# mojing1999/jmcodec

Hardware: AMD Instinct MI355X
Metric: decoded frames/sec @1080p H.264 + bit-exact YUV (higher is better)
Workload: dtype u8

## Files before the change

### jmcodec_amd/csrc/intra_lds.hip

```cpp
#include <hip/hip_runtime.h>
#include "jobs.h"
#include "kernels.h"
#include "kernel_common.h"
#include "chain_common.h"
#include "intra_device.h"

namespace jmamd {

__global__ __launch_bounds__(kIBandRows * 16) __attribute__((amdgpu_waves_per_eu(1, 2))) void k_intra_band(const PicParams *pics, int *ctl, int *err) {
    __shared__ __align__(16) uint8_t smem[kIntraSmemBytes];
    const PicParams &pp = pics[blockIdx.y];
    if (!(pp.stages & PS_INTRA_LDS)) return;
    intra_band_body<false>(pp, blockIdx.x >> 1, blockIdx.x & 1, ctl + (size_t)blockIdx.y * kChainStride + kChainIntraRing, smem, nullptr, err + blockIdx.y);
}

bool intra_lds_supported(int mb_w, int mb_h) { return mb_w > 0 && mb_h <= kIBandRows * kDeblockMaxBands; }

void launch_intra_lds(const PicParams *d_pics, int n, int max_mb_h, int *ctl, int *err, hipStream_t st) {
    const int bands = (max_mb_h + kIBandRows - 1) / kIBandRows;
    hipLaunchKernelGGL(k_intra_band, dim3(2 * bands, n), dim3(kIBandRows * 16), 0, st, d_pics, ctl, err);
}

}
```

Before: 15180.

## Prefetch intra macroblock inputs through a register ring and batch band progress publishing

Replaces the generic intra band body with a stage-pipelined version. Per-macroblock records, residuals and neighbour pixels are requested DEPTH wavefront steps ahead into a register ring, hiding global load latency behind reconstruction. Inter-band progress is now published only every PUB steps, which cuts atomic store and wait traffic but makes the band below wait a little longer. It adds register pressure and a more complex synchronisation protocol that has to stay bit-exact.

```diff
diff --git a/jmcodec_amd/csrc/intra_band_sched.h b/jmcodec_amd/csrc/intra_band_sched.h
--- /dev/null
+++ b/jmcodec_amd/csrc/intra_band_sched.h
@@ -0,0 +1,42 @@
+#pragma once
+#include <stdint.h>
+#ifndef JM_HD
+#if defined(__HIPCC__)
+#include <hip/hip_runtime.h>
+#define JM_HD __host__ __device__ __forceinline__
+#else
+#define JM_HD static inline
+#endif
+#endif
+
+namespace jmamd {
+namespace ibs {
+
+constexpr int kRows = 16;
+constexpr int kAllDone = 0x7fffffff;
+
+JM_HD int band_row0(int band) { return band * kRows; }
+JM_HD int band_rows(int mb_h, int band) { const int left = mb_h - band * kRows; return left < 0 ? 0 : (left < kRows ? left : kRows); }
+JM_HD int first_step(int band) { return 2 * band_row0(band); }
+JM_HD int last_step(int mb_w, int mb_h, int band) { return mb_w - 1 + 2 * (band_row0(band) + band_rows(mb_h, band) - 1); }
+
+JM_HD int mb_x(int s, int row) { return s - 2 * row; }
+JM_HD bool has_mb(int s, int row, int mb_w) { const int x = mb_x(s, row); return x >= 0 && x < mb_w; }
+
+JM_HD constexpr int ring_slots(int D) { return D + 1; }
+JM_HD constexpr int slot_of(int s, int first, int D) { return (s - first) % ring_slots(D); }
+JM_HD constexpr int requested_in(int s, int D) { return s + D; }
+constexpr int kMinDepth = 2, kMaxDepth = 3;
+JM_HD int request_x(int s, int row, int mb_w) { const int x = mb_x(s, row); return x < 0 ? 0 : (x < mb_w ? x : mb_w - 1); }
+JM_HD int group_row(int row0, int rows, int g) { return row0 + (g < rows ? g : 0); }
+
+JM_HD int store_step(int xm, int row0) { return xm + 2 * (row0 - 1); }
+JM_HD int need_above(int xm, int row0) { return store_step(xm, row0) + 1; }
+JM_HD bool covers(int v, int t) { return v > t; }
+JM_HD bool publishes(int s, int first, int P) { return (s - first) % P == 0; }
+JM_HD int published_in(int s) { return s; }
+JM_HD int published_after(int s, int first, int P) { return s - (s - first) % P; }
+JM_HD int publish_lag(int t, int first, int P) { return P - (t - first) % P; }
+
+}
+}
diff --git a/jmcodec_amd/csrc/intra_lds.hip b/jmcodec_amd/csrc/intra_lds.hip
--- a/jmcodec_amd/csrc/intra_lds.hip
+++ b/jmcodec_amd/csrc/intra_lds.hip
@@ -4,21 +4,142 @@
 #include "kernel_common.h"
 #include "chain_common.h"
 #include "intra_device.h"
+#include "intra_band_sched.h"
 
 namespace jmamd {
 
-__global__ __launch_bounds__(kIBandRows * 16) __attribute__((amdgpu_waves_per_eu(1, 2))) void k_intra_band(const PicParams *pics, int *ctl, int *err) {
+static_assert(ibs::kRows == kIBandRows, "intra_band_sched.h describes bands of kIBandRows rows");
+
+struct IStage { uint32_t rec, right; uint4 res0, res1, bot; };
+
+template <bool CHROMA>
+__device__ __forceinline__ IStage istage_request(const gbyte *mbs, const gbyte *resid, const gbyte *plane, int pitch, int mb_w, int row, int s, int l) {
+    constexpr int rows_per_mb = CHROMA ? 8 : 16;
+    const int x = ibs::request_x(s, row, mb_w);
+    const int mb = row * mb_w + x, my_row = CHROMA ? (l & 7) : l;
+    IStage st;
+    st.rec = gload1(mbs + (size_t)mb * sizeof(MbRec) + (l & 7) * 4);
+    const gbyte *px = plane + (size_t)(row * rows_per_mb) * pitch + x * 16;
+    const gbyte *rs = resid + (size_t)mb * 768;
+    st.right = gload1(px + (size_t)my_row * pitch + 12);
+    st.bot = gload4(px + (size_t)(rows_per_mb - 1) * pitch);
+    if (CHROMA) { st.res0 = gload4(rs + 512 + l * 16); st.res1 = make_uint4(0, 0, 0, 0); }
+    else { st.res0 = gload4(rs + l * 32); st.res1 = gload4(rs + l * 32 + 16); }
+    return st;
+}
+
+template <int DEPTH, bool CHROMA>
+__device__ __forceinline__ void intra_stage_body(const PicParams &pp, int band, int *prog_pic, int pub, uint8_t *smem, int *err_word) {
+    const int mb_w = pp.mb_w, mb_h = pp.mb_h, pitch = pp.pitch;
+    const int rows = ibs::band_rows(mb_h, band);
+    if (rows <= 0) return;
+    const int row0 = ibs::band_row0(band);
+    int *prog = prog_pic + (CHROMA ? kDeblockMaxBands : 0);
+    const gbyte *resid = (const gbyte *)pp.resid;
+    const gbyte *mbs = (const gbyte *)pp.mbs;
+    ILds lds{smem, kIBandRows + 1};
+    const int g = threadIdx.x >> 4, l = threadIdx.x & 15;
+    const bool active = g < rows;
+    const int row = ibs::group_row(row0, rows, g), lrow = g + 1;
+    if (threadIdx.x < 144) { lds.i4tab()[threadIdx.x] = (uint8_t)i4_table_entry(threadIdx.x >> 4, threadIdx.x & 3, (threadIdx.x >> 2) & 3);
+        ((uint2 *)lds.i4sel())[threadIdx.x] = i4_sel_entry(threadIdx.x >> 4, threadIdx.x & 3, (threadIdx.x >> 2) & 3); }
+    if (!CHROMA && threadIdx.x < 144) ((pk::I8Sel *)lds.i8sel())[threadIdx.x] = pk::i8_sel_entry(threadIdx.x >> 4, threadIdx.x & 15);
+    gbyte *plane = (gbyte *)(cur_plane(pp) + (CHROMA ? pp.chroma_offset : 0));
+    const ICtx cx{plane, pitch};
+    constexpr int rows_per_mb = CHROMA ? 8 : 16;
+    const bool takes_ring = band > 0 && g == 0;
+    const bool gives_ring = active && g == rows - 1 && row < mb_h - 1;
+    const bool pub_wave = __builtin_amdgcn_readfirstlane((int)(threadIdx.x >> 6)) == ((rows - 1) >> 2) && row0 + rows < mb_h;
+    const int s_begin = ibs::first_step(band), s_end = ibs::last_step(mb_w, mb_h, band);
+    const gbyte *above = plane + (size_t)(row0 * rows_per_mb - 1) * pitch + (l & 3) * 4;
+    gbyte *below = plane + (size_t)((row + 1) * rows_per_mb - 1) * pitch + (l & 3) * 4;
+    int known = 0;
+    auto wait_above = [&](int need) {
+        if (band == 0 || threadIdx.x >= 64 || known >= need) return;
+        int spins = 0;
+        while ((known = __hip_atomic_load(&prog[band - 1], __ATOMIC_RELAXED, __HIP_MEMORY_SCOPE_AGENT)) < need && ++spins < kSpinLimit)
+            __builtin_amdgcn_s_sleep(8);
+        if (known < need) { if (l == 0) report_wait_timeout(err_word, CHAIN_ERR_INTRA_TIMEOUT); known = ibs::kAllDone; }
+        asm volatile("" ::: "memory");
+    };
+    auto ring0 = [&](int xm) -> uint32_t * { return (uint32_t *)(CHROMA ? lds.cring(0, xm & 3) : lds.lring(0, xm & 3)); };
+    auto fetch_above = [&](int xm) -> uint32_t { return __hip_atomic_load((const JM_GLOBAL uint32_t *)(above + (size_t)xm * 16), __ATOMIC_RELAXED,
+        __HIP_MEMORY_SCOPE_AGENT); };
+    if (band > 0) {
+        wait_above(ibs::need_above(mb_w > 1 ? 1 : 0, row0));
+        if (takes_ring && l < 8 && (l >> 2) < mb_w) ring0(l >> 2)[l & 3] = fetch_above(l >> 2);
+    }
+    asm volatile("s_waitcnt vmcnt(0) lgkmcnt(0)\n\ts_barrier" ::: "memory");
+    constexpr int kSlots = ibs::ring_slots(DEPTH);
+    IStage st[kSlots];
+#pragma unroll
+    for (int k = 0; k < DEPTH; k++) st[k] = istage_request<CHROMA>(mbs, resid, plane, pitch, mb_w, row, s_begin + k, l);
+    st[DEPTH].rec = st[DEPTH].right = 0; st[DEPTH].res0 = st[DEPTH].res1 = st[DEPTH].bot = make_uint4(0, 0, 0, 0);
+    __builtin_amdgcn_s_waitcnt(0x0f70);
+    uint32_t p_ring = 0;
+    for (int sb = s_begin; sb <= s_end; sb += kSlots) {
+#pragma unroll
+        for (int k = 0; k < kSlots; k++) {
+            const int s = sb + k;
+            if (s > s_end) break;
+            const IStage c = st[ibs::slot_of(k, 0, DEPTH)];
+            const uint32_t c_ring = p_ring;
+            const int x = ibs::mb_x(s, row);
+            if (takes_ring && l < 4 && x >= 1 && x + 1 < mb_w) ring0(x + 1)[l] = c_ring;
+            const int xf = ibs::mb_x(s, row0) + 2;
+            if (band > 0 && xf < mb_w) wait_above(ibs::need_above(xf, row0));
+            if (takes_ring && l < 4 && xf < mb_w) p_ring = fetch_above(xf);
+            st[ibs::slot_of(ibs::requested_in(k, DEPTH), 0, DEPTH)] = istage_request<CHROMA>(mbs, resid, plane, pitch, mb_w, row, ibs::requested_in(s, DEPTH), l);
+            if (active && x >= 0 && x < mb_w) {
+                if (CHROMA) intra_chroma_mb<false>(cx, lds, x, row, lrow, l, g, c.rec, c.res0, c.right, c.bot);
+                else intra_luma_mb<false>(cx, lds, x, row, lrow, l, g, c.rec, c.res0, c.res1, c.right, c.bot);
+            }
+            if (pub_wave) {
+                if (ibs::publishes(s, s_begin, pub)) {
+                    asm volatile("s_waitcnt vmcnt(0)" ::: "memory");
+                    if (gives_ring && l == 0) __hip_atomic_store(&prog[band], ibs::published_in(s), __ATOMIC_RELAXED, __HIP_MEMORY_SCOPE_AGENT);
+                }
+                if (gives_ring && x >= 0 && x < mb_w && l < 4) __hip_atomic_store((JM_GLOBAL uint32_t *)(below + (size_t)x * 16),
+                    ((const uint32_t *)(CHROMA ? lds.cring(lrow, x & 3) : lds.lring(lrow, x & 3)))[l], __ATOMIC_RELAXED, __HIP_MEMORY_SCOPE_AGENT);
+            }
+            asm volatile("s_waitcnt lgkmcnt(0)\n\ts_barrier" ::: "memory");
+        }
+    }
+    if (pub_wave) {
+        asm volatile("s_waitcnt vmcnt(0)" ::: "memory");
+        if (gives_ring && l == 0) __hip_atomic_store(&prog[band], ibs::kAllDone, __ATOMIC_RELAXED, __HIP_MEMORY_SCOPE_AGENT);
+    }
+}
+
+template <int DEPTH>
+__global__ __launch_bounds__(kIBandRows * 16) __attribute__((amdgpu_waves_per_eu(1, 2))) void k_intra_band(const PicParams *pics, int *ctl, int pub, int *err) {
     __shared__ __align__(16) uint8_t smem[kIntraSmemBytes];
     const PicParams &pp = pics[blockIdx.y];
     if (!(pp.stages & PS_INTRA_LDS)) return;
-    intra_band_body<false>(pp, blockIdx.x >> 1, blockIdx.x & 1, ctl + (size_t)blockIdx.y * kChainStride + kChainIntraRing, smem, nullptr, err + blockIdx.y);
+    int *prog = ctl + (size_t)blockIdx.y * kChainStride + kChainIntraRing;
+    if (blockIdx.x & 1) intra_stage_body<DEPTH, true>(pp, blockIdx.x >> 1, prog, pub, smem, err + blockIdx.y);
+    else intra_stage_body<DEPTH, false>(pp, blockIdx.x >> 1, prog, pub, smem, err + blockIdx.y);
 }
 
 bool intra_lds_supported(int mb_w, int mb_h) { return mb_w > 0 && mb_h <= kIBandRows * kDeblockMaxBands; }
 
+#ifndef JM_INTRA_DEPTH
+#define JM_INTRA_DEPTH 2
+#endif
+#ifndef JM_INTRA_PUB
+#define JM_INTRA_PUB 2
+#endif
+constexpr int kIntraDepth = JM_INTRA_DEPTH, kIntraPub = JM_INTRA_PUB;
+static_assert(ibs::kMinDepth == 2 && ibs::kMaxDepth == 3, "launch_intra_lds chooses between the instantiations for depths 2 and 3");
+static_assert(kIntraDepth >= ibs::kMinDepth && kIntraDepth <= ibs::kMaxDepth && kIntraPub >= 1, "depth and period of this build");
+int intra_depth() { return kIntraDepth; }
+int intra_pub() { return kIntraPub; }
+
 void launch_intra_lds(const PicParams *d_pics, int n, int max_mb_h, int *ctl, int *err, hipStream_t st) {
     const int bands = (max_mb_h + kIBandRows - 1) / kIBandRows;
-    hipLaunchKernelGGL(k_intra_band, dim3(2 * bands, n), dim3(kIBandRows * 16), 0, st, d_pics, ctl, err);
+    dim3 grid(2 * bands, n), block(kIBandRows * 16);
+    if (intra_depth() <= 2) hipLaunchKernelGGL((k_intra_band<2>), grid, block, 0, st, d_pics, ctl, intra_pub(), err);
+    else hipLaunchKernelGGL((k_intra_band<3>), grid, block, 0, st, d_pics, ctl, intra_pub(), err);
 }
 
 }
```

New measurement: 15210 (median of 5 runs). No clear change (+0.2%).
